# jdhuang-csm/bayes-drt

Hardware: AMD Instinct MI355X
Metric: HMC log-posterior+grad evals/sec (81 freq x 161 tau-basis) (higher is better)
Workload: dtype f64

## Files before the change

bayes_drt_amd/csrc/bdrt_device.h:

```cpp
#pragma once
#include <hip/hip_runtime.h>
#include <stdint.h>

namespace bdrt {

constexpr int NC = 16;
constexpr size_t SAMPLER_LDS_RESERVE = 6144;
constexpr int NT = 512;
constexpr int NW = NT / 64;
constexpr int NG = NT / NC;
constexpr int MAXB = 3;
constexpr int NRED = 8;
constexpr int MAXBW = 6;
constexpr int MIN_LR = 192;
constexpr double LOG_015 = -1.8971199848858813;

struct DevBlock {
    int K;
    int is_parallel, is_pos;
    int tilesA;
    int tilesL;
    int tilesK;
    int kpairs;
    int rpairsA;
    int rpairsL;
    int o_x, o_ups, o_d;
    int yp_slot;
    double x_scale;
    const double *Af;
    const double *Lf;
    const double *Bk;
    int toep;
    const double *BkA;
    double T[3][2 * MAXBW + 1];
    const double *tg;
    const double *Ad, *At;
    const double *Ld, *Lt;
};

struct DevProblem {
    int nf, nblocks, D;
    int o_err, o_so;
    int outlier_mode, use_x_sum;
    int n_spectra;
    int XR, ZR, LR, npar;
    int toep_all;
    int w3;
    int fast_s1;
    int fast_hw;
    int toepA;
    int tlen;
    const unsigned *tsteps;
    int zrows;
    int XCR;
    int xc_off[MAXB];
    int big;
    int dbg;
    double sigma_min, ups_alpha, ups_beta, induc_scale;
    double so_lambda, so_alpha, so_beta, x_sum_invscale;
    const double *Z;
    const double *w;
    DevBlock blk[MAXB];
};

__host__ __device__ inline size_t lds_doubles(const DevProblem &P)
{
    return (size_t)NC * ((size_t)P.XR + (size_t)P.ZR * (1 + P.npar) + (size_t)P.LR + (size_t)P.XCR + NW * NRED + 32);
}

typedef double d4 __attribute__((ext_vector_type(4)));

__device__ __forceinline__ d4 mfma_f64(double a, double b, d4 c)
{
    return __builtin_amdgcn_mfma_f64_16x16x4f64(a, b, c, 0, 0, 0);
}


__device__ __forceinline__ double lean_rcp(double b)
{
    double r = __builtin_amdgcn_rcp(b);
    double e = __builtin_fma(-b, r, 1.0);
    r = __builtin_fma(r, e, r);
    e = __builtin_fma(-b, r, 1.0);
    return __builtin_fma(r, e, r);
}

__device__ __forceinline__ double fma_sc(double a, double b, double C)
{
#if defined(__HIP_DEVICE_COMPILE__)
    double d;
// ... 140 lines not shown
                if (p0 + i < pairs) {
                    acc0 = mfma_f64(cur[i].x, bx[i], acc0);
                    acc1 = mfma_f64(cur[i].y, by[i], acc1);
                }
            }
        }
        __builtin_amdgcn_sched_barrier(0);
    };
    dv2 a[PF], b[PF];
    if (nchunk > 0) load(a, 0);
    for (int ch = 0; ch < nchunk; ch += 2) {
        step(a, b, ch, ch + 1 < nchunk);
        if (ch + 1 < nchunk) step(b, a, ch + 1, ch + 2 < nchunk);
    }
}

__device__ __forceinline__ void gemm_forward(const double *__restrict__ Mp, int ntiles, int kpairs,
                                             const double *Xs, double *Ys, int wave, int lane)
{
    const int col = lane & 15, kq = lane >> 4;
    for (int t = wave; t < ntiles; t += NW) {
        d4 acc0 = {0.0, 0.0, 0.0, 0.0}, acc1 = {0.0, 0.0, 0.0, 0.0};
        const double2 *mp = reinterpret_cast<const double2 *>(Mp) + ((size_t)t * kpairs) * 64 + lane;
        mfma_stream(mp, kpairs, Xs + kq * NC + col, acc0, acc1);
#pragma unroll
        for (int r = 0; r < 4; ++r) Ys[(16 * t + kq + 4 * r) * NC + col] = acc0[r] + acc1[r];
    }
}

__device__ __forceinline__ void gemm_backward(const double *__restrict__ Mp, int ntiles, int rpairsA, int rpairsL,
                                              const double *Ra, const double *Rl, double *Gs, int wave, int lane)
{
    const int col = lane & 15, kq = lane >> 4;
    const int rp = rpairsA + rpairsL;
    for (int t = wave; t < ntiles; t += NW) {
        d4 acc0 = {0.0, 0.0, 0.0, 0.0}, acc1 = {0.0, 0.0, 0.0, 0.0};
        const double2 *mp = reinterpret_cast<const double2 *>(Mp) + ((size_t)t * rp) * 64 + lane;
        mfma_stream(mp, rpairsA, Ra + kq * NC + col, acc0, acc1);
        mfma_stream(mp + (size_t)rpairsA * 64, rpairsL, Rl + kq * NC + col, acc0, acc1);
#pragma unroll
        for (int r = 0; r < 4; ++r) Gs[(16 * t + kq + 4 * r) * NC + col] = acc0[r] + acc1[r];
    }
}

template <int NQ>
__device__ __forceinline__ void chain_reduce(double (&v)[NQ], double *red, double *out, int tid)
{
    const int lane = tid & 63, wave = tid >> 6;
#pragma unroll
    for (int q = 0; q < NQ; ++q) {
        double x = v[q];
        x += __shfl_xor(x, 16);
        x += __shfl_xor(x, 32);
        if (lane < NC) red[(wave * NRED + q) * NC + lane] = x;
    }
    __syncthreads();
    if (tid < NQ * NC) {
        const int q = tid / NC, c = tid % NC;
        double s = 0.0;
#pragma unroll
        for (int w = 0; w < NW; ++w) s += red[(w * NRED + q) * NC + c];
        out[q * NC + c] = s;
    }
    __syncthreads();
}

enum { S_RINF = 0, S_INDUC, S_SRES, S_AP, S_AR, S_AI, S_D0 , S_XSUM = 15, S_LP = 16, S_TMP = 17 ,
       S_REJ = 25, S_RAW = 26 , S_NSLOT = 32 };

struct TileIO {
    const double *theta;
    long t_sc, t_sj;
    const int *t_off;
    double *grad;
    long g_sc, g_sj;
    double *lp;
    const int *spec;
    int nvalid;
    int jacobian;
    double *Z_hat;
    double *sigma_tot;
    double *params;
    long long *prof;
};

constexpr int UK = 6;
constexpr int UN = 3;

template <bool TOEP>
__device__ inline void logp_grad_tile(const DevProblem &P, const TileIO &io, double *smem)
{
    int tid = threadIdx.x;
    __asm__ volatile("" : "+v"(tid));
    const int lane = tid & 63, wave = tid >> 6;
    const int c = tid & (NC - 1), g = tid >> 4;
    const int nf = P.nf, N2 = 2 * nf;
    const bool valid = c < io.nvalid;
    const int cc = valid ? c : 0;
    const double jac = io.jacobian ? 1.0 : 0.0;

    double *Xs = smem;
    double *Zh = Xs + (size_t)P.XR * NC;
    double *Yp = Zh + (size_t)P.ZR * NC;
    double *Lr = Yp + (size_t)P.ZR * NC * P.npar;
    double *XC = Lr + (size_t)P.LR * NC;
    double *red = XC + (size_t)P.XCR * NC;
    double *sc = red + NW * NRED * NC;
    const bool cache_x = P.XCR > 0;

    const double *th = io.theta + (long)cc * io.t_sc + (io.t_off ? io.t_off[cc] : 0);
    auto TH = [&](int j) -> double { return th[(long)j * io.t_sj]; };
    double *gr = io.grad ? io.grad + (long)cc * io.g_sc : nullptr;
    auto GW = [&](int j, double v) { if (gr && valid) gr[(long)j * io.g_sj] = v; };
    double *pr = io.params ? io.params + (size_t)cc * P.D : nullptr;
    auto PW = [&](int j, double v) { if (pr && valid) pr[j] = v; };

    long long tprev = (io.prof && tid == 0) ? clock64() : 0;
#define BDRT_TILE_PROF(slot) do { if (io.prof && tid == 0) { const long long t_ = clock64(); io.prof[slot] += t_ - tprev; tprev = t_; } } while (0)
    {
        const int which = tid >> 4;
        const int nsc = 6 + 3 * P.nblocks;
        if (which < nsc) {
            int j;
            if (which < 2) j = which;
            else if (which < 6) j = P.o_err + (which - 2);
            else j = P.blk[(which - 6) / 3].o_d + (which - 6) % 3;
            const double raw = exp(TH(j));
            if (which == 0) { sc[S_RINF * NC + c] = 100.0 * raw; sc[(S_RAW + 0) * NC + c] = raw; }
            else if (which == 1) { sc[S_INDUC * NC + c] = raw * P.induc_scale; sc[(S_RAW + 1) * NC + c] = raw; }
            else if (which < 6) { sc[(S_SRES + which - 2) * NC + c] = 0.05 * raw; sc[(S_RAW + which) * NC + c] = raw; }
            else sc[(S_D0 + which - 6) * NC + c] = raw;
        }
        if (tid < NC) { sc[S_LP * NC + c] = 0.0; sc[S_XSUM * NC + c] = 0.0; sc[S_REJ * NC + c] = 0.0; }
    }
    for (int i = tid; i < P.ZR * NC; i += NT) Zh[i] = 0.0;
    __syncthreads();
    BDRT_TILE_PROF(0);

    for (int b = 0; b < P.nblocks; ++b) {
        const DevBlock &B = P.blk[b];
        const int KP = 8 * B.kpairs;
        double *xc = XC + (size_t)P.xc_off[b] * NC;
        double xs2[2] = {0.0, 0.0};
        for (int k0 = g; k0 < KP; k0 += NG * UK) {
            double t_[UK];
#pragma unroll
            for (int u = 0; u < UK; ++u) { const int k = k0 + NG * u; t_[u] = k < B.K ? TH(B.o_x + k) : 0.0; }
#pragma unroll
            for (int u = 0; u < UK; ++u) {
                const int k = k0 + NG * u;
                if (k < KP) {
                    double xr = 0.0;
                    if (k < B.K) {
                        xr = B.is_pos ? exp(t_[u]) : t_[u];
                        xs2[0] += xr;
                        if (B.is_pos) xs2[1] += t_[u];
                        PW(B.o_x + k, xr);
                    }
                    Xs[k * NC + c] = xr * B.x_scale;
                    if (cache_x) xc[(MAXBW + k) * NC + c] = xr;
                }
            }
        }
        if (cache_x && g < MAXBW) {
            xc[g * NC + c] = 0.0;
            xc[(MAXBW + KP + g) * NC + c] = 0.0;
// ... 371 lines not shown
```

bayes_drt_amd/csrc/bdrt_model.hip:

```cpp
#include <algorithm>
#include <cmath>
#include <cstdlib>
#include <cstring>

#include "bdrt_host.h"
#include "bdrt_big.h"

namespace bdrt {

static thread_local std::string g_last_error;
std::atomic<int> g_process_device{-1};

void set_error(const char *fmt, ...)
{
    char buf[1024];
    va_list ap;
    va_start(ap, fmt);
    vsnprintf(buf, sizeof(buf), fmt, ap);
    va_end(ap);
    g_last_error = buf;
}

static inline int cdiv(int a, int b) { return (a + b - 1) / b; }

// ... 211 lines not shown
            LRs = std::max(LRs, std::max(16 * D.blk[b].tilesA, ((dat->K[b] + 2 * MAXBW) + 15) / 16 * 16));
        }
        if (all) {
            int LR3 = LRs;
            for (int b = 0; b < dat->nblocks; ++b) LR3 = std::max(LR3, (3 * (dat->K[b] + 2 * MAXBW) + 15) / 16 * 16);
            D.LR = LR3; D.w3 = 1;
            if (lds_doubles(D) * sizeof(double) + 8192 > 160 * 1024) { D.LR = LRs; D.w3 = 0; }
            if (lds_doubles(D) * sizeof(double) + 8192 > 160 * 1024) all = false;
        }
        if (!all) {
            D.LR = LR0; D.w3 = 0;
            if (lds_doubles(D) * sizeof(double) + 8192 > 160 * 1024) { D.XCR = 0; for (int b = 0; b < MAXB; ++b) D.xc_off[b] = 0; }
        }
        for (int b = 0; b < dat->nblocks; ++b) D.blk[b].toep = all ? 1 : 0;
        D.toep_all = all ? 1 : 0;
        D.fast_s1 = (all && dat->nblocks == 1 && !D.blk[0].is_parallel && !D.use_x_sum &&
                     D.blk[0].x_scale == 1.0 && nf <= 128 && D.blk[0].K <= 32 * UK &&
                     !getenv("BDRT_GENERIC_TILE")) ? 1 : 0;
        if (D.fast_s1 && D.blk[0].tg && nf / 16 == 5 && nf % 16 <= 2 && (D.blk[0].K / 16) % 5 == 0 && D.blk[0].K >= 80 && D.blk[0].K % 16 <= 2 &&
            !getenv("BDRT_STREAM_A")) {
            D.toepA = 1;
            D.tlen = (8 + nf + D.blk[0].K - 1 + 8 + 1) & ~1;
            const size_t nj = D.outlier_mode ? 0 : s1_nj(D.D);
            if ((s1_lds_doubles(D) + (size_t)NC * 32 * nj) * sizeof(double) + SAMPLER_LDS_RESERVE > 160 * 1024) { D.toepA = 0; D.tlen = 0; }
        }
        if (D.fast_s1 && D.blk[0].tg && nf >= 32 && D.blk[0].K >= 32 && !getenv("BDRT_STREAM_A") &&
            (!D.toepA || (getenv("BDRT_TOEP_GEN") && atoi(getenv("BDRT_TOEP_GEN")) != 0)) &&
            !(getenv("BDRT_TOEP_GEN") && atoi(getenv("BDRT_TOEP_GEN")) == 0)) {
            const int toepA0 = D.toepA, tlen0 = D.tlen;
            D.toepA = 2;
            D.tlen = (16 + nf + D.blk[0].K - 1 + 16 + 1) & ~1;
            D.zrows = std::max(2 * ((nf + 3) & ~3), 16 * D.blk[0].tilesA);
            const size_t nj = D.outlier_mode ? 0 : s1_nj(D.D);
            std::vector<unsigned> steps(TOEP_STEP_WORDS);
            bool ok = true;
            for (int dir = 0; dir < 2 && ok; ++dir)
                for (int w = 0; w < 8 && ok; ++w)
                    ok = toep_gen_steps(dir == 0, nf, D.blk[0].K, D.tlen, w, steps.data() + (size_t)(dir * 8 + w) * 2 * TOEP_STEPS) >= 0;
            if (!ok || (s1_lds_doubles(D) + (size_t)NC * 32 * nj) * sizeof(double) + SAMPLER_LDS_RESERVE > 160 * 1024) { D.toepA = toepA0; D.tlen = tlen0; D.zrows = 0; }
            else if (int rc = upload(P, steps, &D.tsteps)) return rc;
        }
        bool hw = all && !D.fast_s1 && nf <= 128 && !getenv("BDRT_GENERIC_TILE") &&
                  (hw_lds_doubles(D) + 64) * sizeof(double) + 4096 <= 160 * 1024;
        for (int b = 0; b < dat->nblocks; ++b) hw = hw && D.blk[b].K <= 32 * UK;
        D.fast_hw = hw ? 1 : 0;
    }
    if (getenv("BDRT_VERBOSE"))
        fprintf(stderr, "bdrt_problem_create: nf=%d blocks=%d D=%d structured_L=%d (per block %d %d %d) fast_s1=%d fast_hw=%d LDS rows X=%d Z=%d x%d L=%d XC=%d -> %zu B\n",
                nf, dat->nblocks, D.D, D.toep_all, toep_ok[0], dat->nblocks > 1 ? toep_ok[1] : -1, dat->nblocks > 2 ? toep_ok[2] : -1,
                D.fast_s1, D.fast_hw, D.XR, D.ZR, 1 + D.npar, D.LR, D.XCR, lds_doubles(D) * sizeof(double));
    if (const char *e = getenv("BDRT_DEBUG_SKIP")) D.dbg = atoi(e);
    if (D.fast_s1 && s1_lds_doubles(D) * sizeof(double) + SAMPLER_LDS_RESERVE > 160 * 1024 &&
        lds_doubles(D) * sizeof(double) + SAMPLER_LDS_RESERVE <= 160 * 1024) { D.fast_s1 = 0; D.toepA = 0; D.tlen = 0; D.zrows = 0; }
    if (D.fast_hw && hw_lds_doubles(D) * sizeof(double) + SAMPLER_LDS_RESERVE > 160 * 1024 &&
        lds_doubles(D) * sizeof(double) + SAMPLER_LDS_RESERVE <= 160 * 1024) D.fast_hw = 0;
    P.lds_bytes = std::max(std::max(lds_doubles(D), D.fast_hw ? hw_lds_doubles(D) : (size_t)0), D.fast_s1 ? s1_lds_doubles(D) : (size_t)0) * sizeof(double);
    D.big = 0;
    if (P.lds_bytes + SAMPLER_LDS_RESERVE > 160 * 1024 || getenv("BDRT_BIG")) {
        D.big = 1;
        D.fast_s1 = 0; D.fast_hw = 0; D.toepA = 0; D.tlen = 0; D.zrows = 0;
        P.lds_bytes = 4096;
        for (int b = 0; b < dat->nblocks; ++b) {
            DevBlock &B = D.blk[b];
            const int K = B.K;
            const double *A = dat->A[b];
            const double *Ls[3] = {dat->L0[b], dat->L1[b], dat->L2[b]};
            int rc;
            if (!B.Ad) {
                std::vector<double> ad((size_t)N2 * K), at((size_t)K * N2);
                for (int r = 0; r < N2; ++r)
                    for (int m = 0; m < K; ++m) { ad[(size_t)r * K + m] = A[(size_t)r * K + m]; at[(size_t)m * N2 + r] = A[(size_t)r * K + m]; }
                if ((rc = upload(P, ad, &B.Ad)) || (rc = upload(P, at, &B.At))) return rc;
            }
            std::vector<double> ld((size_t)3 * K * K), lt((size_t)3 * K * K);
            for (int i = 0; i < 3; ++i)
                for (int r = 0; r < K; ++r)
                    for (int m = 0; m < K; ++m) {
                        ld[((size_t)i * K + r) * K + m] = Ls[i][(size_t)r * K + m];
                        lt[(size_t)m * 3 * K + (size_t)i * K + r] = Ls[i][(size_t)r * K + m];
                    }
            if ((rc = upload(P, ld, &B.Ld)) || (rc = upload(P, lt, &B.Lt))) return rc;
        }
    }
    std::vector<double> w(nf);
    for (int n = 0; n < nf; ++n) w[n] = 2.0 * M_PI * dat->freq[n];
    int rc;
    if ((rc = upload(P, w, &D.w))) return rc;
    BDRT_HIP(hipStreamCreateWithFlags(&P.stream, hipStreamNonBlocking));
    D.n_spectra = 0;
    return 0;
}

static int set_Z(Problem &P, const double *Z, int n_spectra)
{
    const size_t need = (size_t)n_spectra * 2 * P.dev.nf;
    if (need > P.z_capacity) {
        if (P.d_Z) hipFree(P.d_Z);
        BDRT_HIP(hipMalloc((void **)&P.d_Z, need * sizeof(double)));
        P.z_capacity = need;
    }
    BDRT_HIP(hipMemcpy(P.d_Z, Z, need * sizeof(double), hipMemcpyHostToDevice));
    P.dev.Z = P.d_Z;
    P.dev.n_spectra = n_spectra;
    return P.sync_dev();
}

template <int MODE, int KU = 6>
__global__ __launch_bounds__(NT) void logp_grad_kernel(const DevProblem *__restrict__ Pp, const double *theta, const int *spec, int B,
                                                       int jacobian, double *lp, double *grad, double *params,
                                                       double *Zhat, double *sig)
{
    extern __shared__ __attribute__((aligned(16))) double smem[];
    const DevProblem &P = *Pp;
    if (MODE == 4 || MODE == 6) s1_toep_init(P, smem);
    for (int c0 = blockIdx.x * NC; c0 < B; c0 += gridDim.x * NC) {
        TileIO io;
        io.theta = theta + (size_t)c0 * P.D;
        io.t_sc = P.D; io.t_sj = 1; io.t_off = nullptr;
        io.grad = grad ? grad + (size_t)c0 * P.D : nullptr;
        io.g_sc = P.D; io.g_sj = 1;
        io.lp = lp ? lp + c0 : nullptr;
        io.spec = spec ? spec + c0 : nullptr;
        io.nvalid = min(NC, B - c0);
        io.jacobian = jacobian;
        io.Z_hat = Zhat ? Zhat + (size_t)c0 * 2 * P.nf : nullptr;
        io.sigma_tot = sig ? sig + (size_t)c0 * 2 * P.nf : nullptr;
        io.params = params ? params + (size_t)c0 * P.D : nullptr;
        io.prof = nullptr;
        if (MODE == 4) logp_grad_tile_s1<false, 32, NoHook, NoHook, 1, KU>(P, io, smem);
        else if (MODE == 6) logp_grad_tile_s1<false, 32, NoHook, NoHook, 2, KU>(P, io, smem);
        else if (MODE == 3) logp_grad_tile_hw<KU>(P, io, smem);
        else if (MODE == 2) logp_grad_tile_s1<false, 32, NoHook, NoHook, 0, KU>(P, io, smem);
        else if (MODE == 1) logp_grad_tile<true>(P, io, smem);
        else logp_grad_tile<false>(P, io, smem);
    }
}

__global__ __launch_bounds__(1024) void logp_grad_kernel_wide(const DevProblem *__restrict__ Pp, const double *theta, const int *spec,
                                                              int B, int jacobian, double *lp, double *grad, double *params,
                                                              double *Zhat, double *sig)
{
    extern __shared__ __attribute__((aligned(16))) double smem[];
    const DevProblem &P = *Pp;
    const int c0 = blockIdx.x * NC;
    TileIO io;
    io.theta = theta + (size_t)c0 * P.D;
    io.t_sc = P.D; io.t_sj = 1; io.t_off = nullptr;
    io.grad = grad ? grad + (size_t)c0 * P.D : nullptr;
    io.g_sc = P.D; io.g_sj = 1;
    io.lp = lp ? lp + c0 : nullptr;
    io.spec = spec ? spec + c0 : nullptr;
    io.nvalid = min(NC, B - c0);
    io.jacobian = jacobian;
    io.Z_hat = Zhat ? Zhat + (size_t)c0 * 2 * P.nf : nullptr;
    io.sigma_tot = sig ? sig + (size_t)c0 * 2 * P.nf : nullptr;
    io.params = params ? params + (size_t)c0 * P.D : nullptr;
    io.prof = nullptr;
    logp_grad_tile_s1<false, 64>(P, io, smem);
}

int launch_logp_grad(Problem *p, const double *d_theta, const int *d_spec, int B, int jacobian, double *d_lp,
                     double *d_grad, double *d_params, double *d_Zhat, double *d_sig, hipStream_t stream)
{
    if (B <= 0) return 0;
    BDRT_HIP(hipSetDevice(p->device));
    if (p->dev.big) {
        const int grid = std::min(B, 1024);
        std::lock_guard<std::mutex> lock(p->bigws_mu);
        if (!p->bigws_done) BDRT_HIP(hipEventCreateWithFlags(&p->bigws_done, hipEventDisableTiming));
        else BDRT_HIP(hipStreamWaitEvent(stream, p->bigws_done, 0));
        if (int rc = p->ensure_bigws((size_t)grid * big_ws_doubles(p->dev))) return rc;
        hipLaunchKernelGGL(big_eval_kernel, dim3(grid), dim3(BIG_NT), 0, stream, (const DevProblem *)p->d_dev, p->d_bigws, d_theta, d_spec, B,
                           jacobian, d_lp, d_grad, d_params, d_Zhat, d_sig);
        BDRT_HIP(hipGetLastError());
        BDRT_HIP(hipEventRecord(p->bigws_done, stream));
        return 0;
    }
    static LdsAttrCache attr_cache;
    BDRT_HIP(attr_cache.ensure(p->lds_bytes, [&]() {
        const void *fns[17] = {(const void *)logp_grad_kernel<0>, (const void *)logp_grad_kernel<1>, (const void *)logp_grad_kernel<2>,
                               (const void *)logp_grad_kernel_wide, (const void *)logp_grad_kernel<3>, (const void *)logp_grad_kernel<4>,
// ... 245 lines not shown
```

bayes_drt_amd/csrc/bdrt_nuts16.h:

```cpp
#pragma once
#include <cmath>
#include <cstring>
#include <type_traits>

#include "bdrt_host.h"
#include "bdrt_lbfgs.h"
#include "bdrt_nuts_device.h"
#include "bdrt_solo.h"
#include "bdrt_wave.h"
#include "bdrt_nuts_args.h"
#include "bdrt_big.h"

namespace bdrt {

constexpr int MAXD = 10;
constexpr int NQ_CHK = 2 * MAXD + 2;
static_assert(NW * NQ_CHK * NC <= MIN_LR * NC, "Lr buffer too small for the NUTS reduction scratch");

enum { V_TH = 0, V_P, V_G, V_THM, V_PM, V_GM, V_THP, V_PP, V_GP, V_THS, V_GS, V_THQ, V_GQ, V_RHO, V_MINV,
       V_WMEAN, V_WM2, V_ZN ,
       V_TH2 , V_CKC , V_CKP = V_CKC + MAXD , V_COUNT = V_CKP + MAXD };

__host__ __device__ __forceinline__ int slot_col(int k) { return 2 * (k & 7) + (k >> 3); }
__host__ __device__ __forceinline__ int col_slot(int c) { return (c & 1) * 8 + (c >> 1); }

__device__ __forceinline__ double half_sum(double x) { return sum32(x); }

__device__ __forceinline__ void lds_wave_sync()
{
    __builtin_amdgcn_fence(__ATOMIC_RELEASE, "wavefront");
    __builtin_amdgcn_wave_barrier();
    __builtin_amdgcn_fence(__ATOMIC_ACQUIRE, "wavefront");
}


#include "bdrt_nuts_wide.h"
#include "bdrt_solo_wide.h"
#include "bdrt_lbfgs_dev.h"

#ifndef BDRT_DEEP_VARIANT
#define BDRT_DEEP_VARIANT 1
#endif
#ifndef BDRT_PRE1
#define BDRT_PRE1 0
#endif
#ifndef BDRT_GLDS
#define BDRT_GLDS 0
#endif
#ifndef BDRT_NUTS_ABLATE
#define BDRT_NUTS_ABLATE 0
#endif
#ifndef BDRT_RESIDENT
#define BDRT_RESIDENT 1
#endif
#ifndef BDRT_NT
#define BDRT_NT 1
#endif
#ifndef BDRT_KARG_RELOAD
#define BDRT_KARG_RELOAD 1
#endif
#ifndef BDRT_NUTS_EARLY_STATE
#define BDRT_NUTS_EARLY_STATE 1
#endif
template <int NJ, int MODE, int TA = 0, bool PROF = false>
__global__ __launch_bounds__(NT) void nuts_kernel(const DevProblem *__restrict__ Pp, NutsParams np, NutsArgs a)
{
    extern __shared__ __attribute__((aligned(16))) double smem[];
    const DevProblem &P = *Pp;
    const int tid = threadIdx.x, lane = tid & 63, wave = tid >> 6;
    int c = 2 * wave + (lane >> 5);
    int l32 = lane & 31;
    const int D = P.D, DS = a.ds;
    const int wg = blockIdx.x;
    const int *su = a.slot_unit + (size_t)wg * NC;
    const int kslot = col_slot(c);
    const int unit = su[kslot];
    const bool valid = unit >= 0;

    const size_t tile_doubles = MODE == 4 ? hw_lds_doubles(P) : (MODE >= 2 ? s1_lds_doubles(P) : lds_doubles(P));
    constexpr int DSL = 32 * NJ;
    double *thl = smem + tile_doubles;
    double *lpn = thl + (MODE == 2 ? (size_t)NC * DSL : 0);
    double *hvk = lpn + NC;
    ChainState *sts = reinterpret_cast<ChainState *>(hvk + 2 * NC);
    int *spec = reinterpret_cast<int *>(sts + NC);
    volatile int *slow = spec + NC;
    int *thoff = spec + NC + 4;
    int *hvy = thoff + NC;
    double *ublk = reinterpret_cast<double *>(hvy + NC);
    constexpr bool SPEC = NJ > 16 || (NJ > 11 && MODE < 2);
    const int TH2OFF = (V_TH2 - V_TH) * NC * DS;

    double *V = a.vecs + (size_t)wg * V_COUNT * NC * DS;
    auto row = [&](int v) -> double * { return V + ((size_t)v * NC + c) * DS; };

    static_assert(!TA || MODE >= 2, "the generator table belongs to the S1 tile");
    constexpr int KUX = TA == 0 ? 6 : TA;
    if (TA && MODE == 2) s1_toep_init(P, smem);
    if (tid < NC) {
        const int u = su[col_slot(tid)];
        if (u >= 0) chain_state_copy(sts[tid], a.states[u]);
        else { memset(&sts[tid], 0, sizeof(ChainState)); sts[tid].phase = PH_DONE; }
        spec[tid] = u >= 0 ? sts[tid].spec : 0;
        thoff[tid] = (SPEC && sts[tid].thsel) ? TH2OFF : 0;
        if (tid == 0) *slow = 0;
    }
    __syncthreads();
    ChainState &s = sts[c];
    const Philox rng = {np.seed_lo, np.seed_hi, (uint32_t)s.chain_id};

    TileIO io;
    io.theta = V + (size_t)V_TH * NC * DS; io.t_sc = DS; io.t_sj = 1;
    io.t_off = SPEC ? thoff : nullptr;
    io.grad = V + (size_t)V_G * NC * DS; io.g_sc = DS; io.g_sj = 1;
    if (MODE == 2) {
        io.theta = thl; io.t_sc = DSL;
        io.grad = nullptr;
    }
    io.lp = lpn;
    io.spec = spec;
    io.nvalid = NC;
    io.jacobian = 1;
    io.Z_hat = nullptr; io.sigma_tot = nullptr; io.params = nullptr;
    io.prof = (PROF && a.prof) ? a.prof + (size_t)wg * 32 : nullptr;
    long long tnp = 0;
#define BDRT_NUTS_PROF(slot) do { if (!BDRT_PROF_FINE && io.prof && tid == 0) { const long long t_ = clock64(); io.prof[slot] += t_ - tnp; tnp = t_; } } while (0)
    long long twv = 0;
#define BDRT_WAVE_PROF(slot) do { if (io.prof && lane == 0) { const long long t_ = clock64(); atomicAdd((unsigned long long *)&io.prof[slot], (unsigned long long)(t_ - twv)); twv = t_; } } while (0)

#ifndef BDRT_PROF_FINE
#define BDRT_PROF_FINE 0
#endif
    long long tfn = 0;
    typedef __attribute__((address_space(3))) unsigned long long *lds_u64;
    const lds_u64 fine = (lds_u64)(unsigned long long *)hvk;
    if (BDRT_PROF_FINE && tid < 2 * NC) fine[tid] = 0ull;
#define BDRT_FINE(slot) do { if (BDRT_PROF_FINE && io.prof && lane == 0) { const long long t_ = clock64(); __hip_atomic_fetch_add(&fine[slot], (unsigned long long)(t_ - tfn), __ATOMIC_RELAXED, __HIP_MEMORY_SCOPE_WORKGROUP); tfn = t_; } } while (0)
#define BDRT_FINE_COUNT(slot, cond) do { if (BDRT_PROF_FINE && io.prof) { const bool w_ = __builtin_amdgcn_ballot_w64(cond) != 0; if (lane == 0 && w_) __hip_atomic_fetch_add(&fine[slot], 1ull, __ATOMIC_RELAXED, __HIP_MEMORY_SCOPE_WORKGROUP); } } while (0)
    const int ndbg = BDRT_NUTS_ABLATE ? P.dbg : 0;
    unsigned long long my_leaps = 0;
    double *TH = row(V_TH) + (SPEC && s.thsel ? TH2OFF : 0), *Pm = row(V_P), *G = row(V_G), *MI = row(V_MINV);

    if (!s.kicked) {
        const int ph = s.phase;
        const double e = ph == PH_EPS ? s.eps : (ph == PH_TREE ? s.dir * s.eps : 0.0);
        if (ph == PH_INIT || ph == PH_EPS || ph == PH_TREE) {
            for (int j = l32; j < D; j += 32) {
                const double p = Pm[j] + 0.5 * e * G[j];
                Pm[j] = p;
                TH[j] += e * MI[j] * p;
            }
        }
        s.kicked = 1;
    }
    if (MODE == 2) {
        double *thr = thl + (size_t)c * DSL;
        for (int j = l32; j < DSL; j += 32) thr[j] = j < D ? TH[j] : 0.0;
        TH = thr;
        G = s1_grad_row(P, smem, c);
    }
    constexpr bool FREE_RUN = MODE == 2 && !SPEC;
    int *actf = hvy;
    int any_act;
    {
        const int ph = s.phase;
        const bool running = ph == PH_INIT || ph == PH_EPS || ph == PH_TREE;
        if (FREE_RUN && l32 == 0) actf[c] = running ? 1 : 0;
        any_act = __syncthreads_or(running);
    }

    int ph_c = 0, leaf_c = 0;
    double e_c = 0.0;
    auto refresh_carried = [&]() {
        ph_c = s.phase; leaf_c = s.leaf;
        e_c = ph_c == PH_EPS ? s.eps : (ph_c == PH_TREE ? s.dir * s.eps : 0.0);
    };
    if constexpr (!SPEC) refresh_carried();
    constexpr bool RESIDENT = BDRT_RESIDENT && MODE == 2 && !SPEC && NJ <= 11;
    constexpr int NR = RESIDENT ? NJ : 1;
    double pr_[NR], mir_[NR];
    if constexpr (RESIDENT) {
#pragma unroll
        for (int m = 0; m < NJ; ++m) { const int j = l32 + 32 * m; pr_[m] = valid ? Pm[j] : 0.0; mir_[m] = valid ? MI[j] : 1.0; }
    }

    struct KArgs { const DevProblem *Pp; NutsParams np; NutsArgs a; };
    typedef const __attribute__((address_space(4))) KArgs *kargs_ptr;
    kargs_ptr ka = (kargs_ptr)__builtin_amdgcn_kernarg_segment_ptr();
    const int n_rounds = a.rounds;
    for (int round = 0; round < n_rounds; ++round) {
#if BDRT_KARG_RELOAD
        __asm__ volatile("" : "+s"(ka));
        const NutsParams &np = *(const NutsParams *)&ka->np;
        const NutsArgs &a = *(const NutsArgs *)&ka->a;
#endif
        __asm__ volatile("" : "+v"(c), "+v"(l32));
        if (SPEC && tid < NC) hvy[tid] = 0;
        int ph0;
        double e;
        if constexpr (SPEC) {
            ph0 = s.phase;
            e = ph0 == PH_EPS ? s.eps : (ph0 == PH_TREE ? s.dir * s.eps : 0.0);
        } else { ph0 = ph_c; e = e_c; }
        const bool act = ph0 == PH_INIT || ph0 == PH_EPS || ph0 == PH_TREE;
        if (!any_act) break;
        if (io.prof && tid == 0) tnp = clock64();
        if (io.prof && lane == 0) twv = clock64();

        constexpr int NA = SPEC ? 1 : NJ;
        constexpr int MSAFE = MODE != 2 ? 0 : (NJ == 6 ? 4 : (NJ == 7 ? 6 : (NJ == 11 ? 7 : (NJ == 16 ? 11 : 0))));
        double p_[NA], g_[NA], mi_[NA];
#pragma unroll
        for (int m = 0; m < NA; ++m) { p_[m] = 0.0; g_[m] = 0.0; mi_[m] = 1.0; }
        if constexpr (RESIDENT) {
#pragma unroll
            for (int m = 0; m < NJ; ++m) { p_[m] = pr_[m]; mi_[m] = mir_[m]; }
        }
        auto load_state = [&]() {
            if constexpr (!SPEC && !RESIDENT) {
                if (act) {
#pragma unroll
                    for (int m = 0; m < NJ; ++m) { const int j = l32 + 32 * m; p_[m] = Pm[j]; mi_[m] = MI[j]; }
                }
            }
        };
        int any_next = 0;
        if (MODE == 2) {
            auto read_flags = [&]() {
                if constexpr (FREE_RUN) {
                    typedef int iv4 __attribute__((ext_vector_type(4)));
                    typedef const __attribute__((address_space(3))) iv4 *lds_i4;
                    int v = 0;
#pragma unroll
                    for (int q = 0; q < NC / 4; ++q) { const iv4 f = ((lds_i4)actf)[q]; v |= f.x | f.y | f.z | f.w; }
                    any_next = v;
                }
            };
            constexpr bool EARLY = BDRT_NUTS_EARLY_STATE && NJ <= 11;
            auto early_state = [&]() { if constexpr (EARLY) load_state(); };
            constexpr int KU = NJ <= 4 ? 2 : (NJ <= 6 ? 3 : (NJ <= 7 ? 4 : 6));
            logp_grad_tile_s1<true, 32, decltype(early_state), decltype(read_flags), TA, KU>(P, io, smem, early_state, read_flags);
            if constexpr (!EARLY) load_state();
        }
        else if (MODE == 3) { logp_grad_tile_s1<false, 32, NoHook, NoHook, 0, KUX>(P, io, smem); load_state(); }
        else if (MODE == 4) { logp_grad_tile_hw<KUX, PROF>(P, io, smem); load_state(); }
        else { logp_grad_tile<MODE == 1>(P, io, smem); load_state(); }
        if (io.prof && tid == 0) tnp = clock64();
        BDRT_WAVE_PROF(17);
        const long long t_post0 = (io.prof && SPEC) ? clock64() : 0;
        if constexpr (SPEC) {
            const int dir_now = s.dir;
            const int leaf_now = s.leaf;
            (void)dir_now;
            constexpr int MB = NJ % 8 == 0 ? 8 : 9;
            static_assert(NJ % MB == 0, "chunk size must divide NJ");
            constexpr int NS2 = (32 * NJ + 63) / 64;
            constexpr int LMAX = 4;
            typedef double dv2 __attribute__((ext_vector_type(2)));
            auto ld2 = [](const double *q) -> dv2 { return *reinterpret_cast<const dv2 *>(q); };
            auto st2 = [](double *q, dv2 v) { *reinterpret_cast<dv2 *>(q) = v; };
            if (act) {
                const bool treeph = ph0 == PH_TREE;
                int nmf = 0;
                if (treeph) { while ((leaf_now >> nmf) & 1) ++nmf; }
                const bool lastf = treeph && leaf_now == s.nleaves - 1;
                if (treeph && !lastf && nmf <= LMAX) {
                    const double *RLp[LMAX], *PLp[LMAX];
#pragma unroll
                    for (int l = 0; l < LMAX; ++l) {
                        RLp[l] = l < nmf ? row(l == 0 ? V_CKP : V_CKC + l) : Pm;
                        PLp[l] = l < nmf ? row(V_CKP + l) : Pm;
                    }
                    double *RHD = row(V_CKC + (nmf > 0 ? nmf : 1)), *FRD = row(V_CKP + nmf);
                    double *THN = row(V_TH) + (s.thsel ? 0 : TH2OFF);
                    double kin = 0.0, nonfin = 0.0;
                    double uma[LMAX], umb[LMAX];
#pragma unroll
                    for (int l = 0; l < LMAX; ++l) { uma[l] = 0.0; umb[l] = 0.0; }
                    auto pass = [&](auto nlc, auto sbc) {
                        constexpr int NL = decltype(nlc)::value, SBM = decltype(sbc)::value;
                        auto chunk = [&](int sb, auto sbn) {
                            constexpr int SB = decltype(sbn)::value;
                            dv2 a_[SB], b_[SB], c_[SB], t_[SB], lr_[NL > 0 ? NL : 1][SB], lp_[NL > 0 ? NL : 1][SB];
#pragma unroll
                            for (int ss = 0; ss < SB; ++ss) {
                                {
                                    const int j = 2 * l32 + 64 * (sb + ss);
                                    const int jc = j < DS ? j : 0;
                                    a_[ss] = ld2(Pm + jc); b_[ss] = ld2(G + jc); c_[ss] = ld2(MI + jc); t_[ss] = ld2(TH + jc);
#pragma unroll
                                    for (int l = 0; l < NL; ++l) {
                                        lp_[l][ss] = ld2(PLp[l] + jc);
                                        if (l > 0) lr_[l][ss] = ld2(RLp[l] + jc);
                                    }
                                }
                            }
#pragma unroll
                            for (int ss = 0; ss < SB; ++ss) {
                                {
                                    const int j = 2 * l32 + 64 * (sb + ss);
                                    dv2 pn2, tn2, rho2, first2;
#pragma unroll
                                    for (int hh = 0; hh < 2; ++hh) {
                                        const double p = a_[ss][hh] + 0.5 * e * b_[ss][hh];
                                        const double pn = p + 0.5 * e * b_[ss][hh];
                                        const bool live = j + hh < D;
                                        pn2[hh] = pn;
                                        tn2[hh] = t_[ss][hh] + e * c_[ss][hh] * pn;
                                        if (live) {
                                            kin += c_[ss][hh] * p * p;
                                            nonfin += isfinite(b_[ss][hh]) ? 0.0 : 1.0;
                                        }
// ... 464 lines not shown
                        lds_wave_sync();
                    }
                    double kin0 = 0.0;
                    double pn_[NJ];
#pragma unroll
                    for (int m = 0; m < NJ; ++m) {
                        const int j = l32 + 32 * m;
                        const double p = j < D ? z_[m] / sqrt(mi_[m]) : 0.0;
                        pn_[m] = p;
                        kin0 += mi_[m] * p * p;
                    }
                    kin0 = half_sum(kin0);
                    s.H0 = -s.lps + 0.5 * kin0;
                    if (next == 1) {
                        s.lsw = 0.0; s.lsw_sub = -INFINITY; s.depth = 0; s.leaf = 0; s.nleaves = 1;
                        s.n_leap_iter = 0; s.sum_metro = 0.0;
                        s.dir = rng_uniform(rng, 0, RNG_DIRECTION, 0, 0, (uint32_t)s.iter) > 0.5 ? 1 : -1;
                    }
                    const double e1 = next == 1 ? s.dir * s.eps : s.eps;
                    double *rTHM = row(V_THM), *rTHP = row(V_THP), *rPM = row(V_PM), *rPP = row(V_PP), *rGM = row(V_GM),
                           *rGP = row(V_GP), *rRHO = row(V_RHO);
#pragma unroll
                    for (int m = 0; m < NJ; ++m) {
                        const int j = l32 + 32 * m;
                        const double p = pn_[m];
                        if (next == 1) {
                            rTHM[j] = ths_[m]; rTHP[j] = ths_[m];
                            rPM[j] = p; rPP[j] = p;
                            rGM[j] = gs_[m]; rGP[j] = gs_[m];
                            rRHO[j] = p;
                        }
                        const double pk = p + 0.5 * e1 * gs_[m];
                        if constexpr (RESIDENT) p_[m] = pk; else Pm[j] = pk;
                        TH[j] = ths_[m] + e1 * mi_[m] * pk;
                    }
                } else if (next == 2) {
                    const int dir = s.dir;
                    const double e1 = dir * s.eps;
                    double et_[NJ], ep_[NJ], eg_[NJ];
                    if (dir == dir_now) {
                        if constexpr (GLDS) load_grad(g_);
#pragma unroll
                        for (int m = 0; m < NJ; ++m) { const int j = l32 + 32 * m; et_[m] = TH[j]; ep_[m] = p_[m]; eg_[m] = g_[m]; }
                    } else {
                        const double *ET = row(dir > 0 ? V_THP : V_THM), *EP = row(dir > 0 ? V_PP : V_PM), *EG = row(dir > 0 ? V_GP : V_GM);
#pragma unroll
                        for (int m = 0; m < NJ; ++m) { const int j = l32 + 32 * m; et_[m] = ET[j]; ep_[m] = EP[j]; eg_[m] = EG[j]; }
                    }
#pragma unroll
                    for (int m = 0; m < NJ; ++m) {
                        const int j = l32 + 32 * m;
                        const double pk = ep_[m] + 0.5 * e1 * eg_[m];
                        if constexpr (RESIDENT) p_[m] = pk; else Pm[j] = pk;
                        TH[j] = et_[m] + e1 * mi_[m] * pk;
                    }
                } else if (next == 4) {
#pragma unroll
                    for (int m = 0; m < NJ; ++m) {
                        const int j = l32 + 32 * m;
                        if (j < D) {
                            TH[j] = np.init_radius * (2.0 * rng_uniform(rng, (uint32_t)j, RNG_INIT, 0, att, 0) - 1.0);
                            if constexpr (RESIDENT) p_[m] = 0.0; else Pm[j] = 0.0;
                        }
                    }
                }
            }
        }
        BDRT_FINE(12);
        BDRT_NUTS_PROF(15);
        BDRT_NUTS_PROF(16);

        BDRT_WAVE_PROF(22);
        if (io.prof && lane == 0 && next) atomicAdd((unsigned long long *)&io.prof[24], 1ull);
        if constexpr (RESIDENT) {
#pragma unroll
            for (int m = 0; m < NJ; ++m) { pr_[m] = p_[m]; mir_[m] = mi_[m]; }
        }
        {
            if (cont) leaf_c = leaf_now + 1; else refresh_carried();
            const int ph = ph_c;
            const bool running = ph == PH_INIT || ph == PH_EPS || ph == PH_TREE;
            if constexpr (FREE_RUN) {
                if (l32 == 0) actf[c] = running ? 1 : 0;
                any_act = any_next;
            } else {
                any_act = __syncthreads_or(running);
            }
        }
        BDRT_WAVE_PROF(23);
        BDRT_NUTS_PROF(10);
        }
    }

    __syncthreads();
    if (BDRT_PROF_FINE && io.prof && tid < 17) atomicAdd((unsigned long long *)&io.prof[tid], (unsigned long long)fine[tid]);
    if (MODE == 2) {
        double *THg = row(V_TH);
        for (int j = l32; j < D; j += 32) THg[j] = TH[j];
    }
    if constexpr (RESIDENT) {
        if (valid) {
#pragma unroll
            for (int m = 0; m < NJ; ++m) { const int j = l32 + 32 * m; Pm[j] = pr_[m]; }
        }
    }
    if (l32 == 0 && valid) chain_state_copy(a.states[unit], s);
    {
        unsigned long long x = my_leaps;
        x += __shfl_xor(x, 32);
        if (lane == 0 && x) atomicAdd(a.leap_counter, x);
    }
    {
        const int ph = s.phase;
        const bool running = ph == PH_INIT || ph == PH_EPS || ph == PH_TREE;
        const int busy = __syncthreads_or(running);
        if (tid == 0 && !busy) atomicAdd(a.done_counter, 1);
        if (a.active_counter && l32 == 0 && running && valid) atomicAdd(a.active_counter, 1);
    }
}

#define BDRT_NUTS16_G0(X) X(11, 2, 1) X(11, 2, 2) X(11, 2, 0) X(4, 2, 2) X(4, 2, 0) X(6, 2, 1)
#define BDRT_NUTS16_G1(X) X(16, 2, 2) X(16, 2, 1) X(16, 2, 0) X(6, 2, 2) X(6, 2, 0) X(7, 2, 2) X(7, 2, 0)
#define BDRT_NUTS16_G2(X) X(11, 1, 0) X(11, 0, 0) X(16, 1, 0) X(16, 0, 0) X(27, 1, 0) X(27, 0, 0)
#define BDRT_NUTS16_G3(X) X(11, 3, 0) X(16, 3, 0) X(11, 3, 3) X(16, 3, 3) X(11, 3, 4) X(16, 3, 4)
#define BDRT_NUTS16_G4(X) X(11, 4, 0) X(16, 4, 0) X(27, 4, 0) X(11, 4, 3) X(16, 4, 3) X(27, 4, 3) X(11, 4, 4) X(16, 4, 4) X(27, 4, 4)
#define BDRT_NUTS16_G5(X) X(11, 2, 1) X(11, 2, 2) X(7, 2, 2) X(27, 4, 0)
#define BDRT_NUTS16_DEFINE(NJ_, MODE_, TA_) template __global__ void nuts_kernel<NJ_, MODE_, TA_, false>(const DevProblem *__restrict__, NutsParams, NutsArgs);
#define BDRT_NUTS16_DECLARE(NJ_, MODE_, TA_) extern template __global__ void nuts_kernel<NJ_, MODE_, TA_, false>(const DevProblem *__restrict__, NutsParams, NutsArgs);
#define BDRT_NUTS16_DEFINE_PROF(NJ_, MODE_, TA_) template __global__ void nuts_kernel<NJ_, MODE_, TA_, true>(const DevProblem *__restrict__, NutsParams, NutsArgs);
#define BDRT_NUTS16_DECLARE_PROF(NJ_, MODE_, TA_) extern template __global__ void nuts_kernel<NJ_, MODE_, TA_, true>(const DevProblem *__restrict__, NutsParams, NutsArgs);

}
```

bayes_drt_amd/csrc/bdrt_tile_s1.h:

```cpp
#pragma once
#include "bdrt_device.h"
#include <type_traits>

namespace bdrt {

static __device__ long long *g_tile_trace = nullptr;

__device__ __forceinline__ int swz(int row, int col) { return row * NC + (col ^ (row & 15)); }

template <int LPC>
__device__ __forceinline__ double hsum(double x)
{
    x = sum32(x);
    if (LPC == 64) x += __shfl_xor(x, 32);
    return x;
}

__device__ __forceinline__ void wave_sync()
{
    __builtin_amdgcn_fence(__ATOMIC_RELEASE, "wavefront");
    __builtin_amdgcn_wave_barrier();
    __builtin_amdgcn_fence(__ATOMIC_ACQUIRE, "wavefront");
}

// ... 604 lines not shown
    long long *trc = g_tile_trace ? g_tile_trace + ((size_t)blockIdx.x * NWV + wave) * 16 : nullptr;
#define BDRT_S1_TRACE(slot) do { if (trc && (lane == 0)) trc[slot] = clock64(); } while (0)
    BDRT_S1_TRACE(0);
#define BDRT_S1_PROF(slot) do { if (io.prof && tid == 0) { const long long t_ = clock64(); io.prof[slot] += t_ - tprev; tprev = t_; } } while (0)
    long long twe = io.prof ? clock64() : 0;
#define BDRT_S1_BARRIER(slot, wslot) do { if (io.prof) { const long long tb_ = clock64(); __syncthreads(); const long long te_ = clock64(); \
        if (lane == 0) { atomicAdd((unsigned long long *)&io.prof[slot], (unsigned long long)(te_ - tb_)); \
                         if (wslot) atomicAdd((unsigned long long *)&io.prof[wslot], (unsigned long long)(tb_ - twe)); } \
        twe = te_; } else __syncthreads(); } while (0)

    double sraw = 0.0, st = 0.0;
    {
        int j = -1;
        if (l32 < 2) j = l32;
        else if (l32 < 6) j = P.o_err + (l32 - 2);
        else if (l32 < 9) j = B.o_d + (l32 - 6);
        if (j >= 0) { st = TH(j); sraw = lean_exp(st); PW(j, sraw); }
    }
    double lp = 0.0;
    int lp_lane = -1;
    double x_[UKV];
    {
        double tx_[UKV], tu_[UKV];
#pragma unroll
        for (int u = 0; u < UKV; ++u) {
            const int k = l32 + LPC * u, kk = k < K ? k : 0;
            tx_[u] = TH(B.o_x + kk);
            tu_[u] = TH(B.o_ups + kk);
        }
#pragma unroll
        for (int u = 0; u < UKV; ++u) {
            const bool in = l32 + LPC * u < K;
            tx_[u] = in ? tx_[u] : 0.0;
            tu_[u] = in ? tu_[u] : 0.0;
        }
        double ex_[UKV];
#pragma unroll
        for (int u = 0; u < UKV; ++u) ex_[u] = lean_exp(tx_[u]);
#pragma unroll
        for (int u = 0; u < UKV; ++u) {
            const int k = l32 + LPC * u;
            double xr = 0.0;
            if (k < K) {
                xr = B.is_pos ? ex_[u] : tx_[u];
                if (B.is_pos) lp += jac * tx_[u];
                PW(B.o_x + k, xr);
            }
            x_[u] = xr;
            if (k < KP) Xs[swz(k, c)] = xr;
            xrow[MAXBW + k] = xr;
            wrow[MAXBW + k] = tu_[u];
        }
        if (l32 < MAXBW) {
            xrow[l32] = 0.0; xrow[MAXBW + LPC * UKV + l32] = 0.0;
            wrow[l32] = 0.0; wrow[MAXBW + LPC * UKV + l32] = 0.0;
        }
    }
    static_assert(!TA || LPC == 32, "the Toeplitz-A GEMMs are written for 512 threads");
    const double *Tt = TA ? s1_toep_table(P, smem) : nullptr;
    const int tlen = TA ? P.tlen : 0;
    constexpr int TPAD = toep_pad<TA>();
    const int nfi = toep_im_row<TA>(nf);
    if (TA) {
        const int r16 = TA == 2 ? toep_gen_odd(nf) : (nf & 15), n0 = nf - r16;
        for (int j = 0; j < r16; ++j) {
            double sr = 0.0, si = 0.0;
#pragma unroll
            for (int u = 0; u < UKV; ++u) {
                const int idx = max(TPAD + n0 + j + (K - 1) - (l32 + LPC * u), 0);
                sr = fma(Tt[idx], x_[u], sr); si = fma(Tt[tlen + idx], x_[u], si);
            }
            sr = hsum<LPC>(sr); si = hsum<LPC>(si);
            if (l32 == 0) { Zh[swz(n0 + j, c)] = sr; Zh[swz(nfi + n0 + j, c)] = si; }
        }
        if (TA == 2) toep_zero_split_gen<true>(nf, K, Zh, tid); else toep_zero_split<true>(nf, K, Zh, tid);
    }
    const double d0 = __shfl(sraw, hb | 6), d1 = __shfl(sraw, hb | 7), d2 = __shfl(sraw, hb | 8);
    const double israw5 = 5.0 * lean_rcp(sraw);
    if (l32 < 6) lp += -0.5 * sraw * sraw + jac * st;
    else if (l32 < 9) lp += -6.0 * st - israw5 + jac * st;
#ifndef BDRT_SPEC_EARLY
#define BDRT_SPEC_EARLY 0
#endif
#ifndef BDRT_EARLY_P2
#define BDRT_EARLY_P2 1
#endif
#ifndef BDRT_TOEP_PREFETCH
#define BDRT_TOEP_PREFETCH 1
#endif
#ifndef BDRT_P2_OPAQUE_K
#define BDRT_P2_OPAQUE_K 1
#endif
    constexpr bool EARLY_P2 = BDRT_EARLY_P2 != 0;
    double zre_[UNV], zim_[UNV], wn_[UNV];
    auto load_spectrum = [&]() {
        const int sp = io.spec ? io.spec[cc] : 0;
        const double *Zm = P.Z + (size_t)sp * N2;
#pragma unroll
        for (int v = 0; v < UNV; ++v) {
            const int n = l32 + LPC * v, nn = n < nf ? n : 0;
            zre_[v] = Zm[nn]; zim_[v] = Zm[nf + nn]; wn_[v] = P.w[nn];
        }
    };
#pragma unroll 1
    for (int step = 0; step < 2; ++step) {
    if (EARLY_P2 ? step == 1 : step == 0) {
        BDRT_S1_TRACE(1);
        ToepLane tlane;
        if (TA == 1 && BDRT_TOEP_PREFETCH) tlane = toep_lane_fetch<true>(K, tlen, Tt, wave, lane);
        BDRT_S1_BARRIER(25, 29);
        after_x_ready();
        if constexpr (BDRT_SPEC_EARLY) load_spectrum();
        BDRT_S1_TRACE(2);
        BDRT_S1_PROF(1);
        BDRT_S1_TRACE(3);
        if (!(dbg & 1)) {
            if (TA == 2) toep_gemm_gen<true>(nf, K, tlen, Tt, Xs, Zh, wave, lane);
            else if (TA) {
                if (!BDRT_TOEP_PREFETCH) tlane = toep_lane_fetch<true>(K, tlen, Tt, wave, lane);
                toep_gemm<true>(nf, K, tlen, Tt, wave, lane, tlane);
            }
            else gemm_sw<NWV, GPFV>(B.Af, B.tilesA, B.kpairs, Xs, Zh, wave, lane);
        }
        continue;
    }

    BDRT_S1_TRACE(4);
    if (!(dbg & 4)) {
        const int kb = UKV * l32;
        double xw[WINV], tuc[UKV];
#pragma unroll
        for (int j = 0; j < WINV; ++j) xw[j] = xrow[kb + j];
#pragma unroll
        for (int u = 0; u < UKV; ++u) tuc[u] = wrow[MAXBW + kb + u];
        wave_sync();
        double v0_[UKV], v1_[UKV], v2_[UKV];
#pragma unroll
        for (int u = 0; u < UKV; ++u) { v0_[u] = 0.0; v1_[u] = 0.0; v2_[u] = 0.0; }
        double tn0 = B.T[0][0], tn1 = B.T[1][0], tn2 = B.T[2][0];
#pragma unroll
        for (int d = 0; d < NTAP; ++d) {
            const double t0 = tn0, t1 = tn1, t2 = tn2;
            if (d + 1 < NTAP) { tn0 = B.T[0][d + 1]; tn1 = B.T[1][d + 1]; tn2 = B.T[2][d + 1]; }
            __asm__ volatile("" ::: "memory");
#pragma unroll
            for (int u = 0; u < UKV; ++u) { v0_[u] = fma(t0, xw[u + d], v0_[u]); v1_[u] = fma(t1, xw[u + d], v1_[u]); v2_[u] = fma(t2, xw[u + d], v2_[u]); }
        }
        double ue[UKV + 4], ie[UKV + 2];
#pragma unroll
        for (int u = 0; u < UKV; ++u) { ue[u + 2] = 0.15 * lean_exp(tuc[u]); ie[u + 1] = lean_rcp(ue[u + 2]); }
        {
            const int lo = hb | ((l32 + LPC - 1) & (LPC - 1)), hi = hb | ((l32 + 1) & (LPC - 1));
            ue[0] = __shfl(ue[UKV], lo); ue[1] = __shfl(ue[UKV + 1], lo);
            ue[UKV + 2] = __shfl(ue[2], hi); ue[UKV + 3] = __shfl(ue[3], hi);
            ie[0] = __shfl(ie[UKV], lo); ie[UKV + 1] = __shfl(ie[1], hi);
        }
        BDRT_S1_PROF(5);
        double sv0 = 0, sv1 = 0, sv2 = 0;
        double w0_[UKV], w1_[UKV], w2_[UKV], gup[UKV];
#pragma unroll
        for (int u = 0; u < UKV; ++u) {
            int k = kb + u;
#if BDRT_P2_OPAQUE_K
            __asm__ volatile("" : "+v"(k));
#endif
            w0_[u] = 0.0; w1_[u] = 0.0; w2_[u] = 0.0; gup[u] = 0.0;
            if (k < K) {
                const double um2 = ue[u], um1 = ue[u + 1], uu = ue[u + 2], up1 = ue[u + 3], up2 = ue[u + 4];
                const double t = tuc[u];
                const double iu = ie[u + 1], iu2 = iu * iu;
                const double v0 = v0_[u], v1 = v1_[u], v2 = v2_[u];
                const double q2 = d0 * v0 * v0 + d1 * v1 * v1 + d2 * v2 * v2;
                const double ir = 0.15 * iu;
                lp += -(t + LOG_015) - 0.5 * q2 * iu2 - (P.ups_alpha + 1.0) * t - P.ups_beta * ir + jac * t;
                sv0 += v0 * v0 * iu2; sv1 += v1 * v1 * iu2; sv2 += v2 * v2 * iu2;
                double gu = -iu + q2 * iu2 * iu;
                if (k >= 1 && k + 1 < K) {
                    const double du = 0.5 * (uu - 0.5 * (um1 + up1)) * iu;
// ... 108 lines not shown
            const double h_re = -0.5 * w_re + 0.5 * e_re * e_re * w_re * w_re;
            const double h_im = -0.5 * w_im + 0.5 * e_im * e_im * w_im * w_im;
            const double gzr = e_re * w_re + 2.0 * zr * (h_re * (ap2 + ar2) + h_im * ar2);
            const double gzi = e_im * w_im + 2.0 * zi * (h_im * (ap2 + ai2) + h_re * ai2);
            Zh[swz(n, c)] = gzr;
            Zh[swz(nfi + n, c)] = gzi;
            if (TA && rk > 0) {
                lk0 = fma(tk0r_[v], gzr, fma(tk0i_[v], gzi, lk0));
                if (rk > 1) lk1 = fma(tk1r_[v], gzr, fma(tk1i_[v], gzi, lk1));
            }
            sR += gzr;
            sL += gzi * wn;
            sH += h_re + h_im;
            sHz2 += h_re * zr * zr + h_im * zi * zi;
            sHzr2 += (h_re + h_im) * zr * zr;
            sHzi2 += (h_re + h_im) * zi * zi;
            if (omode == 1) {
                const double dso = 2.0 * so_re * (h_re + h_im);
                GW(P.o_so + n, r0 * (0.05 * r1 * dso - P.so_lambda) + jac);
                GW(P.o_so + nf + n, 0.05 * r0 * r1 * dso - (P.so_alpha + 1.0) + P.so_beta / r1 + jac);
                lp += -P.so_lambda * r0 - (P.so_alpha + 1.0) * t1 - P.so_beta / r1 + jac * (t0 + t1);
            } else if (omode == 2) {
                GW(P.o_so + n, r0 * (0.05 * 2.0 * so_re * h_re - P.so_lambda) + jac);
                GW(P.o_so + nf + n, r1 * (0.05 * 2.0 * so_im * h_im - P.so_lambda) + jac);
                lp += -P.so_lambda * (r0 + r1) + jac * (t0 + t1);
            }
            if (!LDSIO && io.Z_hat && valid) { io.Z_hat[(size_t)c * N2 + n] = zr; io.Z_hat[(size_t)c * N2 + nf + n] = zi; }
            if (!LDSIO && io.sigma_tot && valid) {
                io.sigma_tot[(size_t)c * N2 + n] = sqrt(s2_re);
                io.sigma_tot[(size_t)c * N2 + nf + n] = sqrt(s2_im);
            }
        }
        lp += -0.5 * lean_log(pp_lo);
        if (nf > LPC * (UNV / 2)) lp += -0.5 * lean_log(pp_hi);
        double dl = 0.0;
        if constexpr (LPC == 32) {
            const double q[8] = {sR, sL, sH, sHz2, sHzr2, sHzi2, lk0, lp};
            const double tot = sum32_by_lane<8>(q, l32);
            dl = (l32 == 0 ? 100.0 : (l32 == 1 ? P.induc_scale : 0.005 * sraw)) * tot;
            if (TA && rk > 0) {
                if (l32 == 6) Xs[swz(K - rk, c)] = tot;
                if (rk > 1) { lk1 = hsum<LPC>(lk1); if (l32 == 0) Xs[swz(K - rk + 1, c)] = lk1; }
            }
            lp = tot;
            lp_lane = 7;
        } else {
            sR = hsum<LPC>(sR); sL = hsum<LPC>(sL); sH = hsum<LPC>(sH); sHz2 = hsum<LPC>(sHz2); sHzr2 = hsum<LPC>(sHzr2); sHzi2 = hsum<LPC>(sHzi2);
            if (l32 == 0) dl = 100.0 * sR;
            else if (l32 == 1) dl = P.induc_scale * sL;
            else if (l32 == 2) dl = 0.05 * 2.0 * s_res * sH;
            else if (l32 == 3) dl = 0.05 * 2.0 * a_p * sHz2;
            else if (l32 == 4) dl = 0.05 * 2.0 * a_r * sHzr2;
            else dl = 0.05 * 2.0 * a_i * sHzi2;
        }
        if (l32 < 6) {
            const int j = l32 < 2 ? l32 : P.o_err + (l32 - 2);
            gsc = sraw * (dl - sraw) + jac;
            GW(j, gsc);
        }
    }
    BDRT_S1_TRACE(7);
    ToepLane tlane;
    if (TA == 1 && BDRT_TOEP_PREFETCH) tlane = toep_lane_fetch<false>(K, tlen, Tt, wave, lane);
    BDRT_S1_BARRIER(27, 31);
    BDRT_S1_TRACE(8);
    BDRT_S1_PROF(4);
    before_backward();
    if (!(dbg & 2)) {
        if (TA == 2) toep_gemm_gen<false>(nf, K, tlen, Tt, Zh, Xs, wave, lane);
        else if (TA) {
            if (!BDRT_TOEP_PREFETCH) tlane = toep_lane_fetch<false>(K, tlen, Tt, wave, lane);
            toep_gemm<false>(nf, K, tlen, Tt, wave, lane, tlane);
        }
        else gemm_sw<NWV, GPFV>(B.BkA, B.tilesK, B.rpairsA, Zh, Xs, wave, lane);
    }
    BDRT_S1_TRACE(9);
    BDRT_S1_BARRIER(28, 0);
    BDRT_S1_TRACE(10);
    BDRT_S1_PROF(8);

    double gx_[UKV], gu_[UKV];
    {
        double ag_[UKV], gl2_[UKV];
#pragma unroll
        for (int u = 0; u < UKV; ++u) {
            const int k = l32 + LPC * u, kk = k < K ? k : 0;
            ag_[u] = Xs[swz(kk, c)]; gl2_[u] = wrow[MAXBW + k]; gu_[u] = xrow[MAXBW + k];
        }
#pragma unroll
        for (int u = 0; u < UKV; ++u) {
            const int k = l32 + LPC * u;
            const double graw = ag_[u] + gl2_[u];
            const double gx = B.is_pos ? x_[u] * graw + jac : graw;
            gx_[u] = k < K ? gx : 0.0;
            gu_[u] = k < K ? gu_[u] : 0.0;
            if (!LDSIO && k < K) { GW(B.o_x + k, gx_[u]); GW(B.o_ups + k, gu_[u]); }
        }
    }
    if (LDSIO) {
        wave_sync();
#pragma unroll
        for (int u = 0; u < UKV; ++u) {
            const int k = l32 + LPC * u;
            if (k < K) { xrow[B.o_x + k] = gx_[u]; xrow[B.o_ups + k] = gu_[u]; }
        }
        if (l32 < 9) xrow[l32 < 2 ? l32 : (l32 < 6 ? P.o_err + (l32 - 2) : B.o_d + (l32 - 6))] = gsc;
    }
    if (lp_lane < 0) { lp = hsum<LPC>(lp); lp_lane = 0; }
    if (l32 == lp_lane && io.lp && valid) io.lp[c] = lp;
    BDRT_S1_PROF(9);
    BDRT_S1_TRACE(11);
    if (LDSIO) wave_sync(); else __syncthreads();
}

__device__ __forceinline__ double *s1_grad_row(const DevProblem &P, double *smem, int c)
{
    return smem + (size_t)NC * (P.XR + s1_zrows(P)) + (size_t)c * (2 * RW);
}

}
```

Baseline: 175.2 million.

## Pad spectra buffers and use lane-based addressing for spectrum and epilogue loads

Pads the frequency and impedance device buffers with zeroed slack so the spectrum loader can read unconditionally from a per-chain byte offset, using global address-space pointers instead of clamped indices. The gradient epilogue gets the same treatment, with one lane base pointer plus constant strides for the Xs, wrow and xrow loads. The NUTS free-run active-flag check now reads the flag per lane and combines it with a wave ballot instead of a vector LDS read. These changes aim to cut address arithmetic and LDS traffic in the hot loop. In exchange they rely on padding invariants, and a new 2 GiB size limit is added for the spectra buffer.

Result: faster. 177.5 million, median of 6 (+1.3%).

```diff
diff --git a/bayes_drt_amd/csrc/bdrt_device.h b/bayes_drt_amd/csrc/bdrt_device.h
--- a/bayes_drt_amd/csrc/bdrt_device.h
+++ b/bayes_drt_amd/csrc/bdrt_device.h
@@ -6,6 +6,7 @@
 
 constexpr int NC = 16;
 constexpr size_t SAMPLER_LDS_RESERVE = 6144;
+constexpr int SPEC_PAD = 128;
 constexpr int NT = 512;
 constexpr int NW = NT / 64;
 constexpr int NG = NT / NC;
@@ -312,6 +313,7 @@
     double *sigma_tot;
     double *params;
     long long *prof;
+    int zoff;
 };
 
 constexpr int UK = 6;
diff --git a/bayes_drt_amd/csrc/bdrt_model.hip b/bayes_drt_amd/csrc/bdrt_model.hip
--- a/bayes_drt_amd/csrc/bdrt_model.hip
+++ b/bayes_drt_amd/csrc/bdrt_model.hip
@@ -317,7 +317,7 @@
             if ((rc = upload(P, ld, &B.Ld)) || (rc = upload(P, lt, &B.Lt))) return rc;
         }
     }
-    std::vector<double> w(nf);
+    std::vector<double> w((size_t)nf + SPEC_PAD, 0.0);
     for (int n = 0; n < nf; ++n) w[n] = 2.0 * M_PI * dat->freq[n];
     int rc;
     if ((rc = upload(P, w, &D.w))) return rc;
@@ -329,9 +329,12 @@
 static int set_Z(Problem &P, const double *Z, int n_spectra)
 {
     const size_t need = (size_t)n_spectra * 2 * P.dev.nf;
+    if ((need + SPEC_PAD) * sizeof(double) >= ((size_t)1 << 31)) { set_error("spectra of one problem must stay below 2 GiB (%d given)", n_spectra); return -1; }
     if (need > P.z_capacity) {
         if (P.d_Z) hipFree(P.d_Z);
-        BDRT_HIP(hipMalloc((void **)&P.d_Z, need * sizeof(double)));
+        P.d_Z = nullptr; P.z_capacity = 0;
+        BDRT_HIP(hipMalloc((void **)&P.d_Z, (need + SPEC_PAD) * sizeof(double)));
+        BDRT_HIP(hipMemset(P.d_Z + need, 0, SPEC_PAD * sizeof(double)));
         P.z_capacity = need;
     }
     BDRT_HIP(hipMemcpy(P.d_Z, Z, need * sizeof(double), hipMemcpyHostToDevice));
diff --git a/bayes_drt_amd/csrc/bdrt_nuts16.h b/bayes_drt_amd/csrc/bdrt_nuts16.h
--- a/bayes_drt_amd/csrc/bdrt_nuts16.h
+++ b/bayes_drt_amd/csrc/bdrt_nuts16.h
@@ -58,6 +58,9 @@
 #endif
 #ifndef BDRT_KARG_RELOAD
 #define BDRT_KARG_RELOAD 1
+#endif
+#ifndef BDRT_FLAGS_BALLOT
+#define BDRT_FLAGS_BALLOT 1
 #endif
 #ifndef BDRT_NUTS_EARLY_STATE
 #define BDRT_NUTS_EARLY_STATE 1
@@ -84,7 +87,8 @@
     double *hvk = lpn + NC;
     ChainState *sts = reinterpret_cast<ChainState *>(hvk + 2 * NC);
     int *spec = reinterpret_cast<int *>(sts + NC);
-    volatile int *slow = spec + NC;
+    typedef volatile __attribute__((address_space(3))) int *lds_vint;
+    lds_vint slow = (lds_vint)(spec + NC);
     int *thoff = spec + NC + 4;
     int *hvy = thoff + NC;
     double *ublk = reinterpret_cast<double *>(hvy + NC);
@@ -119,6 +123,7 @@
     }
     io.lp = lpn;
     io.spec = spec;
+    io.zoff = MODE == 2 ? spec[c] * (2 * P.nf * (int)sizeof(double)) : 0;
     io.nvalid = NC;
     io.jacobian = 1;
     io.Z_hat = nullptr; io.sigma_tot = nullptr; io.params = nullptr;
@@ -225,9 +230,12 @@
             }
         };
         int any_next = 0;
+        int flag_l = 0;
         if (MODE == 2) {
             auto read_flags = [&]() {
-                if constexpr (FREE_RUN) {
+                if constexpr (FREE_RUN && BDRT_FLAGS_BALLOT) {
+                    flag_l = ((const __attribute__((address_space(3))) int *)actf)[l32 & (NC - 1)];
+                } else if constexpr (FREE_RUN) {
                     typedef int iv4 __attribute__((ext_vector_type(4)));
                     typedef const __attribute__((address_space(3))) iv4 *lds_i4;
                     int v = 0;
@@ -858,6 +866,7 @@
             const bool running = ph == PH_INIT || ph == PH_EPS || ph == PH_TREE;
             if constexpr (FREE_RUN) {
                 if (l32 == 0) actf[c] = running ? 1 : 0;
+                if constexpr (BDRT_FLAGS_BALLOT) any_next = __builtin_amdgcn_ballot_w64(flag_l != 0) != 0 ? 1 : 0;
                 any_act = any_next;
             } else {
                 any_act = __syncthreads_or(running);
diff --git a/bayes_drt_amd/csrc/bdrt_tile_s1.h b/bayes_drt_amd/csrc/bdrt_tile_s1.h
--- a/bayes_drt_amd/csrc/bdrt_tile_s1.h
+++ b/bayes_drt_amd/csrc/bdrt_tile_s1.h
@@ -710,6 +710,12 @@
 #ifndef BDRT_SPEC_EARLY
 #define BDRT_SPEC_EARLY 0
 #endif
+#ifndef BDRT_SPEC_GLOBAL
+#define BDRT_SPEC_GLOBAL 1
+#endif
+#ifndef BDRT_EPI_LANE_BASE
+#define BDRT_EPI_LANE_BASE 1
+#endif
 #ifndef BDRT_EARLY_P2
 #define BDRT_EARLY_P2 1
 #endif
@@ -722,6 +728,16 @@
     constexpr bool EARLY_P2 = BDRT_EARLY_P2 != 0;
     double zre_[UNV], zim_[UNV], wn_[UNV];
     auto load_spectrum = [&]() {
+        if constexpr (LDSIO && BDRT_SPEC_GLOBAL) {
+            static_assert(LPC * UNV <= SPEC_PAD, "P.w / P.Z are padded by SPEC_PAD doubles");
+            typedef const __attribute__((address_space(1))) double *gptr;
+            typedef const __attribute__((address_space(1))) char *gbytes;
+            const unsigned l8 = 8u * (unsigned)l32, z8 = (unsigned)io.zoff + l8;
+            const gptr wl = (gptr)((gbytes)P.w + l8), zr = (gptr)((gbytes)P.Z + z8), zi = (gptr)((gbytes)(P.Z + nf) + z8);
+#pragma unroll
+            for (int v = 0; v < UNV; ++v) { zre_[v] = zr[LPC * v]; zim_[v] = zi[LPC * v]; wn_[v] = wl[LPC * v]; }
+            return;
+        }
         const int sp = io.spec ? io.spec[cc] : 0;
         const double *Zm = P.Z + (size_t)sp * N2;
 #pragma unroll
@@ -996,10 +1012,19 @@
     double gx_[UKV], gu_[UKV];
     {
         double ag_[UKV], gl2_[UKV];
-#pragma unroll
-        for (int u = 0; u < UKV; ++u) {
-            const int k = l32 + LPC * u, kk = k < K ? k : 0;
-            ag_[u] = Xs[swz(kk, c)]; gl2_[u] = wrow[MAXBW + k]; gu_[u] = xrow[MAXBW + k];
+        if constexpr (BDRT_EPI_LANE_BASE) {
+            static_assert(LPC % 16 == 0 && LPC * UKV <= 2 * RW, "rows l32 + LPC u of Xs: same swizzle, inside the workgroup's LDS");
+            int le = l32;
+            __asm__ volatile("" : "+v"(le));
+            const double *xs0 = Xs + swz(le, c), *w0 = wrow + MAXBW + le, *x0 = xrow + MAXBW + le;
+#pragma unroll
+            for (int u = 0; u < UKV; ++u) { ag_[u] = xs0[LPC * NC * u]; gl2_[u] = w0[LPC * u]; gu_[u] = x0[LPC * u]; }
+        } else {
+#pragma unroll
+            for (int u = 0; u < UKV; ++u) {
+                const int k = l32 + LPC * u, kk = k < K ? k : 0;
+                ag_[u] = Xs[swz(kk, c)]; gl2_[u] = wrow[MAXBW + k]; gu_[u] = xrow[MAXBW + k];
+            }
         }
 #pragma unroll
         for (int u = 0; u < UKV; ++u) {
```
